# brain-research/l2hmc

Hardware: AMD Instinct MI355X
Metric: chain_leapfrog_steps_per_sec (higher is better)
Workload: dtype f32

## Files before the change

### l2hmc_amd/csrc/traj_fast.hpp

```cpp
#pragma once
#include "l2hmc_kernels.hpp"
#include "bf3k.hpp"


namespace l2hmc {

__device__ __forceinline__ float relu_i(float a) { return __int_as_float(max(__float_as_int(a), 0)); }
__device__ __forceinline__ f4 rcp4(f4 a) {
  return f4{__builtin_amdgcn_rcpf(a.x), __builtin_amdgcn_rcpf(a.y), __builtin_amdgcn_rcpf(a.z),
            __builtin_amdgcn_rcpf(a.w)};
}
__device__ __forceinline__ f4 ex2_4(f4 a) {
  return f4{__builtin_amdgcn_exp2f(a.x), __builtin_amdgcn_exp2f(a.y), __builtin_amdgcn_exp2f(a.z),
            __builtin_amdgcn_exp2f(a.w)};
}

typedef _Float16 h2v __attribute__((ext_vector_type(2)));
typedef _Float16 h8v __attribute__((ext_vector_type(8)));
typedef float f2v __attribute__((ext_vector_type(2)));
#define L2HMC_F16_SCALE 64.0f
struct WF16 {
  h8v a1;
  h8v a2;
};
__device__ __forceinline__ h2v cvt_pk16(float a, float b) { return __builtin_convertvector(f2v{a, b}, h2v); }
__device__ __forceinline__ h2v lo_pair16(h2v h, float a0, float a1) {
  h2v r;
  const float ns = -L2HMC_F16_SCALE;
  asm("v_fma_mixlo_f16 %0, %1, %2, %3 op_sel:[0,0,0] op_sel_hi:[1,0,0]" : "=v"(r) : "v"(h), "s"(ns), "v"(a0));
  asm("v_fma_mixhi_f16 %0, %1, %2, %3 op_sel:[1,0,0] op_sel_hi:[1,0,0]" : "+v"(r) : "v"(h), "s"(ns), "v"(a1));
  return r;
}
template <bool LAT>
__device__ __forceinline__ h8v split16(f4 a) {
  const f4 ad = a * (1.f / L2HMC_F16_SCALE);
  const h2v h01 = cvt_pk16(ad.x, ad.y), h23 = cvt_pk16(ad.z, ad.w);
  h2v l01, l23;
  if constexpr (LAT) {
    float r0, r1, r2, r3;
    const float ns = -L2HMC_F16_SCALE;
    asm("v_fma_mix_f32 %0, %1, %2, %3 op_sel:[0,0,0] op_sel_hi:[1,0,0]" : "=v"(r0) : "v"(h01), "s"(ns), "v"(a.x));
    asm("v_fma_mix_f32 %0, %1, %2, %3 op_sel:[1,0,0] op_sel_hi:[1,0,0]" : "=v"(r1) : "v"(h01), "s"(ns), "v"(a.y));
    asm("v_fma_mix_f32 %0, %1, %2, %3 op_sel:[0,0,0] op_sel_hi:[1,0,0]" : "=v"(r2) : "v"(h23), "s"(ns), "v"(a.z));
    asm("v_fma_mix_f32 %0, %1, %2, %3 op_sel:[1,0,0] op_sel_hi:[1,0,0]" : "=v"(r3) : "v"(h23), "s"(ns), "v"(a.w));
    l01 = cvt_pk16(r0, r1);
    l23 = cvt_pk16(r2, r3);
  } else {
    l01 = lo_pair16(h01, a.x, a.y);
    l23 = lo_pair16(h23, a.z, a.w);
  }
  return h8v{h01.x, h01.y, h23.x, h23.y, l01.x, l01.y, l23.x, l23.y};
}
__device__ __forceinline__ WF16 wsplit16(f4 w) {
  const float sc = L2HMC_F16_SCALE;
  const h2v h01 = cvt_pk16(w.x, w.y), h23 = cvt_pk16(w.z, w.w);
  const f4 r = f4{w.x - (float)h01.x, w.y - (float)h01.y, w.z - (float)h23.x, w.w - (float)h23.y} * sc;
  const h2v L01 = cvt_pk16(r.x, r.y), L23 = cvt_pk16(r.z, r.w);
  const h2v H01 = cvt_pk16((float)h01.x * sc, (float)h01.y * sc), H23 = cvt_pk16((float)h23.x * sc, (float)h23.y * sc);
  const h2v l01 = cvt_pk16((float)L01.x / sc, (float)L01.y / sc), l23 = cvt_pk16((float)L23.x / sc, (float)L23.y / sc);
  WF16 f;
  f.a1 = h8v{H01.x, H01.y, H23.x, H23.y, h01.x, h01.y, h23.x, h23.y};
  f.a2 = h8v{L01.x, L01.y, L23.x, L23.y, l01.x, l01.y, l23.x, l23.y};
  return f;
}
#define L2HMC_F16_STATE_MAX 2.5e5f
__device__ __forceinline__ float amax4(f4 a) { return fmaxf(fmaxf(fabsf(a.x), fabsf(a.y)), fmaxf(fabsf(a.z), fabsf(a.w))); }
__device__ __forceinline__ f4 mfma16x2(const WF16& W, h8v b, f4 acc) {
  acc = __builtin_amdgcn_mfma_f32_16x16x32_f16(W.a1, b, acc, 0, 0, 0);
  return __builtin_amdgcn_mfma_f32_16x16x32_f16(W.a2, b, acc, 0, 0, 0);
}

__host__ __device__ constexpr int fast_fw_net_f32(int NTp) { return (3 * NTp + 1) * 256; }
__host__ __device__ constexpr int fast_fw_net(int NTp, bool f16 = false) { return (3 * NTp + 1) * (f16 ? 512 : 256); }
__host__ __device__ inline int fast_dpp(int NTp) { return 16 * NTp + 16; }
__host__ __device__ inline int fast_fc_net(int NTp) { return 4 * fast_dpp(NTp); }
__host__ __device__ inline int fast_rec(int NTp) { return 32 + 16 * NTp; }
__host__ __device__ inline int fast_rec_dir(int NTp, int T) { return (T + 2) * fast_rec(NTp) + 16; }

long long plan_lds_fast(KArgs& k, int NW, int DT, bool f16 = false);

#ifndef L2HMC_FAST_SPLIT_LAT_TAIL
#define L2HMC_FAST_SPLIT_LAT_TAIL true
#endif
#ifndef L2HMC_FAST_SPLIT_LAT_PAIR
#define L2HMC_FAST_SPLIT_LAT_PAIR true
#endif
#ifndef L2HMC_FAST_SPLIT_LAT_L1
#define L2HMC_FAST_SPLIT_LAT_L1 false
#endif
template <int DT, bool F16 = false>
struct TailK {
  f4 w2;
  f4 hs[DT], ht[DT], hq[DT];
  f4 cS[DT], cQ[DT], bQ[DT];
};
template <int DT>
struct TailK<DT, true> {
  WF16 w2;
  WF16 hs[DT], ht[DT], hq[DT];
  f4 cS[DT], cQ[DT], bQ[DT];
};

template <int DT>
__device__ __forceinline__ void load_tailk(TailK<DT, false>& tk, const float* fw, const float* fc, int dofs, int NTp,
                                           int w, int lane) {
  const int q = lane >> 4, DPp = fast_dpp(NTp);
  tk.w2 = lds4(fw + lane * 4);
#pragma unroll
  for (int t = 0; t < DT; ++t) {
    const int tg = w * DT + t;
    tk.hs[t] = lds4(fw + ((1 + 3 * tg + 0) * 64 + lane) * 4);
    tk.ht[t] = lds4(fw + ((1 + 3 * tg + 1) * 64 + lane) * 4);
    tk.hq[t] = lds4(fw + ((1 + 3 * tg + 2) * 64 + lane) * 4);
    tk.cS[t] = lds4(fc + dofs + 16 * tg + 4 * q);
    tk.cQ[t] = lds4(fc + 2 * DPp + 16 * tg + 4 * q);
    tk.bQ[t] = lds4(fc + 3 * DPp + 16 * tg + 4 * q);
  }
}
__device__ __forceinline__ WF16 lds_wf16(const float* fw, int NTp, int g, int lane) {
  WF16 f;
  f.a1 = *reinterpret_cast<const h8v*>(fw + (g * 64 + lane) * 4);
  f.a2 = *reinterpret_cast<const h8v*>(fw + (3 * NTp + 1) * 256 + (g * 64 + lane) * 4);
  return f;
}
template <int DT>
__device__ __forceinline__ void load_tailk(TailK<DT, true>& tk, const float* fw, const float* fc, int dofs, int NTp,
                                           int w, int lane) {
  const int q = lane >> 4, DPp = fast_dpp(NTp);
  tk.w2 = lds_wf16(fw, NTp, 0, lane);
#pragma unroll
  for (int t = 0; t < DT; ++t) {
    const int tg = w * DT + t;
    tk.hs[t] = lds_wf16(fw, NTp, 1 + 3 * tg + 0, lane);
    tk.ht[t] = lds_wf16(fw, NTp, 1 + 3 * tg + 1, lane);
    tk.hq[t] = lds_wf16(fw, NTp, 1 + 3 * tg + 2, lane);
    tk.cS[t] = lds4(fc + dofs + 16 * tg + 4 * q);
    tk.cQ[t] = lds4(fc + 2 * DPp + 16 * tg + 4 * q);
    tk.bQ[t] = lds4(fc + 3 * DPp + 16 * tg + 4 * q);
  }
}

template <int DT, int KH, class F>
__device__ __forceinline__ void tail_fast(const TailK<DT, false>& tk, f4 hs_, F&& apply) {
  f4 h = splat(0.f);
#pragma unroll
  for (int r = 0; r < KH; ++r) h[r] = relu_i(hs_[r]);
  {
    f4 acc = splat(0.f);
#pragma unroll
    for (int r = 0; r < KH; ++r) acc = MFMA16(tk.w2[r], h[r], acc);
#pragma unroll
    for (int r = 0; r < KH; ++r) h[r] = relu_i(acc[r]);
  }
#pragma unroll
  for (int t = 0; t < DT; ++t) {
    f4 zs = splat(0.f), zt = splat(0.f), zq = splat(0.f);
#pragma unroll
    for (int r = 0; r < KH; ++r) {
      zs = MFMA16(tk.hs[t][r], h[r], zs);
      zq = MFMA16(tk.hq[t][r], h[r], zq);
      zt = MFMA16(tk.ht[t][r], h[r], zt);
    }
#if !defined(L2HMC_NO_HEAD_FENCE)
    __builtin_amdgcn_sched_barrier(0);
#endif
    const f4 rS = rcp4(-(ex2_4(zs) * 0.5f + 0.5f));
    const f4 aS = rS * tk.cS[t] + tk.cS[t];
    const f4 rQ = rcp4(-(ex2_4(zq) * 0.5f + 0.5f));
    const f4 EQ = ex2_4(rQ * tk.cQ[t] + tk.bQ[t]);
    apply(t, aS, zt, EQ);
  }
}
template <int DT, int KH, class F>
__device__ __forceinline__ void tail_fast(const TailK<DT, true>& tk, f4 hs_, F&& apply) {
  f4 h = splat(0.f);
#pragma unroll
  for (int r = 0; r < KH; ++r) h[r] = relu_i(hs_[r]);
  {
    const f4 acc = mfma16x2(tk.w2, split16<L2HMC_FAST_SPLIT_LAT_TAIL>(h), splat(0.f));
#pragma unroll
    for (int r = 0; r < KH; ++r) h[r] = relu_i(acc[r]);
  }
  const h8v b = split16<L2HMC_FAST_SPLIT_LAT_TAIL>(h);
#pragma unroll
  for (int t = 0; t < DT; ++t) {
    f4 zs = __builtin_amdgcn_mfma_f32_16x16x32_f16(tk.hs[t].a1, b, splat(0.f), 0, 0, 0);
    f4 zq = __builtin_amdgcn_mfma_f32_16x16x32_f16(tk.hq[t].a1, b, splat(0.f), 0, 0, 0);
    f4 zt = __builtin_amdgcn_mfma_f32_16x16x32_f16(tk.ht[t].a1, b, splat(0.f), 0, 0, 0);
    zs = __builtin_amdgcn_mfma_f32_16x16x32_f16(tk.hs[t].a2, b, zs, 0, 0, 0);
    zq = __builtin_amdgcn_mfma_f32_16x16x32_f16(tk.hq[t].a2, b, zq, 0, 0, 0);
    zt = __builtin_amdgcn_mfma_f32_16x16x32_f16(tk.ht[t].a2, b, zt, 0, 0, 0);
    const f4 rS = rcp4(-(ex2_4(zs) * 0.5f + 0.5f));
    const f4 aS = rS * tk.cS[t] + tk.cS[t];
    const f4 rQ = rcp4(-(ex2_4(zq) * 0.5f + 0.5f));
    const f4 EQ = ex2_4(rQ * tk.cQ[t] + tk.bQ[t]);
    apply(t, aS, zt, EQ);
  }
}

template <int DT, int KH, class FA, class FB>
__device__ __forceinline__ void tail_fast2(const TailK<DT, true>& tk, f4 hsa, f4 hsb, FA&& applyA, FB&& keepB) {
  f4 ha = splat(0.f), hb = splat(0.f);
#pragma unroll
  for (int r = 0; r < KH; ++r) { ha[r] = relu_i(hsa[r]); hb[r] = relu_i(hsb[r]); }
  {
    const h8v sa = split16<L2HMC_FAST_SPLIT_LAT_PAIR>(ha), sb = split16<L2HMC_FAST_SPLIT_LAT_PAIR>(hb);
    f4 acca = __builtin_amdgcn_mfma_f32_16x16x32_f16(tk.w2.a1, sa, splat(0.f), 0, 0, 0);
    f4 accb = __builtin_amdgcn_mfma_f32_16x16x32_f16(tk.w2.a1, sb, splat(0.f), 0, 0, 0);
    acca = __builtin_amdgcn_mfma_f32_16x16x32_f16(tk.w2.a2, sa, acca, 0, 0, 0);
    accb = __builtin_amdgcn_mfma_f32_16x16x32_f16(tk.w2.a2, sb, accb, 0, 0, 0);
#pragma unroll
    for (int r = 0; r < KH; ++r) { ha[r] = relu_i(acca[r]); hb[r] = relu_i(accb[r]); }
  }
  const h8v ba = split16<L2HMC_FAST_SPLIT_LAT_PAIR>(ha), bb = split16<L2HMC_FAST_SPLIT_LAT_PAIR>(hb);
#pragma unroll
  for (int t = 0; t < DT; ++t) {
    f4 zsa = __builtin_amdgcn_mfma_f32_16x16x32_f16(tk.hs[t].a1, ba, splat(0.f), 0, 0, 0);
    f4 zqa = __builtin_amdgcn_mfma_f32_16x16x32_f16(tk.hq[t].a1, ba, splat(0.f), 0, 0, 0);
    f4 zta = __builtin_amdgcn_mfma_f32_16x16x32_f16(tk.ht[t].a1, ba, splat(0.f), 0, 0, 0);
    f4 zsb = __builtin_amdgcn_mfma_f32_16x16x32_f16(tk.hs[t].a1, bb, splat(0.f), 0, 0, 0);
    f4 zqb = __builtin_amdgcn_mfma_f32_16x16x32_f16(tk.hq[t].a1, bb, splat(0.f), 0, 0, 0);
    f4 ztb = __builtin_amdgcn_mfma_f32_16x16x32_f16(tk.ht[t].a1, bb, splat(0.f), 0, 0, 0);
    zsa = __builtin_amdgcn_mfma_f32_16x16x32_f16(tk.hs[t].a2, ba, zsa, 0, 0, 0);
    zqa = __builtin_amdgcn_mfma_f32_16x16x32_f16(tk.hq[t].a2, ba, zqa, 0, 0, 0);
    zta = __builtin_amdgcn_mfma_f32_16x16x32_f16(tk.ht[t].a2, ba, zta, 0, 0, 0);
    zsb = __builtin_amdgcn_mfma_f32_16x16x32_f16(tk.hs[t].a2, bb, zsb, 0, 0, 0);
    zqb = __builtin_amdgcn_mfma_f32_16x16x32_f16(tk.hq[t].a2, bb, zqb, 0, 0, 0);
    ztb = __builtin_amdgcn_mfma_f32_16x16x32_f16(tk.ht[t].a2, bb, ztb, 0, 0, 0);
    const f4 rSa = rcp4(-(ex2_4(zsa) * 0.5f + 0.5f));
    const f4 aSa = rSa * tk.cS[t] + tk.cS[t];
    const f4 rQa = rcp4(-(ex2_4(zqa) * 0.5f + 0.5f));
    const f4 EQa = ex2_4(rQa * tk.cQ[t] + tk.bQ[t]);
    applyA(t, aSa, zta, EQa);
    const f4 rSb = rcp4(-(ex2_4(zsb) * 0.5f + 0.5f));
    const f4 aSb = rSb * tk.cS[t] + tk.cS[t];
    const f4 rQb = rcp4(-(ex2_4(zqb) * 0.5f + 0.5f));
    const f4 EQb = ex2_4(rQb * tk.cQ[t] + tk.bQ[t]);
    keepB(t, aSb, ztb, EQb);
  }
}

template <int DT>
struct L1W16 {
  WF16 xa[DT], xb[DT], va[DT], vb[DT];
};
template <int DT>
__device__ __forceinline__ f4 l1_part16(const f4 (&z)[DT], f4 acc, const WF16* W) {
#pragma unroll
  for (int t = 0; t < DT; ++t) acc = mfma16x2(W[t], split16<L2HMC_FAST_SPLIT_LAT_L1>(z[t]), acc);
  return acc;
}

template <int EK, int DT, int NW, int KH, int PK = 0>
#ifndef L2HMC_FAST_WAVES
#define L2HMC_FAST_WAVES 2
#endif
#ifndef L2HMC_FAST_WAVES_DT2
#define L2HMC_FAST_WAVES_DT2 1
#endif
__global__ __launch_bounds__(64 * NW, (DT >= 2 && PK == 1) ? L2HMC_FAST_WAVES_DT2 : L2HMC_FAST_WAVES) void traj_fast_kernel(const KArgs A) {
  extern __shared__ __attribute__((aligned(16))) float smem[];
  lds_poison(smem);
  static_assert(DT <= 2, "the fast kernel keeps layer-1 and tail fragments in registers");
  const int tid = threadIdx.x, lane = tid & 63, nthr = 64 * NW;
  const int w = NW > 1 ? __builtin_amdgcn_readfirstlane(tid >> 6) : 0;
  const int c = lane & 15, q = lane >> 4;
  const long long chain = (long long)blockIdx.x * 16 + c;
  const bool live = chain < A.N;
  const int NT = A.NT, DP = 16 * NT, NF = net_floats(NT);
  const float LOG2E = 1.4426950408889634f;
  const float eps = A.alpha != nullptr ? expf(*A.alpha) : A.eps_host;
  const float heps = 0.5f * eps;
  constexpr int NTp = NW * DT;
  constexpr bool F16 = PK == 1;
  const int FWN = fast_fw_net(NTp, F16), DPp = fast_dpp(NTp), FCN = fast_fc_net(NTp), R = fast_rec(NTp),
            RECD = fast_rec_dir(NTp, A.T);

  {
    constexpr int GN = 3 * NTp + 1;
    constexpr int NCP = 2 * GN * 64, NTRIP = (NCP + 64 * NW - 1) / (64 * NW);
    for (int t0 = 0; t0 < NTRIP; t0 += 8) {
      f4 buf[8];
#pragma unroll
      for (int u = 0; u < 8; ++u) {
        const int i = tid + (t0 + u) * nthr;
        const int net = i >= GN * 64, j = i - net * (GN * 64), g = j >> 6;
        buf[u] = splat(0.f);
        if (i < NCP && g < 3 * NT + 1) buf[u] = reinterpret_cast<const f4*>(A.packed + (size_t)net * NF + (2 * NT + 1) * 256)[j];
      }
#pragma unroll
      for (int u = 0; u < 8; ++u) {
        const int i = tid + (t0 + u) * nthr;
        const int net = i >= GN * 64, j = i - net * (GN * 64), g = j >> 6;
        float sc = 1.f;
        if (g > 0) sc = ((g - 1) % 3 == 1) ? (net == 0 ? eps : heps) : 2.f * LOG2E;
        if constexpr (F16) {
          if (i < NCP) {
            const WF16 f = wsplit16(buf[u] * sc);
            float* base = smem + A.o_fw + net * FWN;
            reinterpret_cast<h8v*>(base)[j] = f.a1;
            reinterpret_cast<h8v*>(base + GN * 256)[j] = f.a2;
          }
        } else {
          if (i < NCP) reinterpret_cast<f4*>(smem + A.o_fw + net * FWN)[j] = buf[u] * sc;
        }
      }
    }
  }
  for (int i = tid; i < 2 * 16 * NTp; i += nthr) {
    const int net = i / (16 * NTp), dim = i % (16 * NTp);
    const float* scl = A.packed + (size_t)net * NF + net_groups(NT) * 256;
    const float epn = net == 0 ? eps : heps;
    const float es = dim < DP ? scl[dim] : 0.f, eq = dim < DP ? scl[DP + dim] : 0.f;
    const float cs = es * epn * LOG2E, cq = eq * eps * LOG2E;
    float* fc = smem + A.o_fc + net * FCN;
    fc[dim] = cs;
    fc[DPp + dim] = -cs;
    fc[2 * DPp + dim] = cq;
    fc[3 * DPp + dim] = cq + log2f(epn);
  }
#pragma unroll 4
  for (int i = tid; i < 2 * A.T * R; i += nthr) {
    const int dr = i / (A.T * R), r = (i / R) % A.T, j = i % R;
    const bool tb = j < 32;
    const int net = tb ? j >> 4 : 0, u = j & 15, dim = tb ? 0 : j - 32;
    const float* tf = A.packed + (size_t)net * NF + (2 * NT * 64) * 4;
    const float a0 = tf[u * 4], a1 = tf[(16 + u) * 4], a2 = tf[(32 + u) * 4], c0 = A.trig[2 * r], c1 = A.trig[2 * r + 1];
    const float mk = A.masks[r * A.d + (dim < A.d ? dim : 0)];
    const float m = dim < A.d ? mk : 0.f;
    smem[A.o_rec + dr * RECD + (r + 1) * R + j] = tb ? fmaf(a0, c0, fmaf(a1, c1, a2)) : (dr ? m : 1.f - m);
  }
  stage_energy<EK, false>(A, smem, tid, nthr);

  f4 x[DT], v[DT], g[DT];
  load_state<DT, NW>(A.x, A, chain, live, w, q, x);
  const bool need_p = A.p_out != nullptr || A.x_next != nullptr || A.u != nullptr ||
                      (A.rng_flags & L2HMC_RNG_U) != 0;
  __syncthreads();

  const float* fwx = smem + A.o_fw;
  const float* fwv = fwx + FWN;
  const float* fcx = smem + A.o_fc;
  const float* fcv = fcx + FCN;
  int pb = 0;
  const f4 Z = splat(0.f);
  EnergyRegs<EK, DT> er;
  load_energy_regs<EK, DT, NW>(er, A, smem, w, lane);
  auto grad = [&](const f4 (&xx)[DT], f4 (&gg)[DT], float& Up, bool wantU) {
    if constexpr (EK == L2HMC_ENERGY_GAUSS_DIAG) {
#pragma unroll
      for (int t = 0; t < DT; ++t) gg[t] = er.prec[t] * (xx[t] - er.mu[t]);
    } else {
      grad_energy<EK, DT, NW>(A, smem, w, lane, xx, gg, Up, wantU, &er);
    }
  };
  auto diag_U = [&](const f4 (&xx)[DT], const f4 (&gg)[DT]) {
    float U = 0.f;
    if constexpr (EK == L2HMC_ENERGY_GAUSS_DIAG) {
#pragma unroll
      for (int t = 0; t < DT; ++t) U += 0.5f * hsum((xx[t] - er.mu[t]) * gg[t]);
    }
    return U;
  };
  float U_start = 0.f;
  grad(x, g, U_start, need_p);
  if constexpr (EK == L2HMC_ENERGY_GAUSS_DIAG) U_start = diag_U(x, g);

  L1W<DT> l1w;
  load_l1w<DT, NW>(l1w, A.packed, A.packed + NF, A, w, lane);
  TailK<DT, F16> tk;
  f4 pv[1];
  L1W16<F16 ? DT : 1> l1h;
  auto vnet_l1 = [&](const f4 (&xx)[DT], const f4 (&gg)[DT]) {
    if constexpr (F16) {
      if constexpr (EK == L2HMC_ENERGY_GAUSS_DIAG) return l1_part16<DT>(xx, Z, l1h.va);
      else return l1_part16<DT>(gg, l1_part16<DT>(xx, Z, l1h.va), l1h.vb);
    } else if constexpr (EK == L2HMC_ENERGY_GAUSS_DIAG) {
      return l1_part<DT, NW>(nullptr, 0, A, w, lane, xx, Z, l1w.va);
    } else {
      return l1_part<DT, NW>(nullptr, 0, A, w, lane, xx, Z, l1w.va) + l1_part<DT, NW>(nullptr, NT, A, w, lane, gg, Z, l1w.vb);
    }
  };
  if constexpr (EK == L2HMC_ENERGY_GAUSS_DIAG) {
    f4 pm[DT], cv[1];
#pragma unroll
    for (int t = 0; t < DT; ++t) {
      l1w.va[t] = l1w.va[t] + er.prec[t] * l1w.vb[t];
      pm[t] = -(er.prec[t] * er.mu[t]);
    }
    cv[0] = l1_part<DT, NW>(nullptr, NT, A, w, lane, pm, Z, l1w.vb);
    xchg<NW, 1>(cv, A, smem, w, lane, pb);
    if (w == 0 && c == 0) {
      for (int i = 0; i < 2 * A.T; ++i) {
        float* tb = smem + A.o_rec + (i / A.T) * RECD + (i % A.T + 1) * R + 16 + 4 * q;
        *reinterpret_cast<f4*>(tb) = lds4(tb) + cv[0];
      }
    }
    __syncthreads();
  }
  if constexpr (F16) {
#pragma unroll
    for (int t = 0; t < DT; ++t) {
      l1h.xa[t] = wsplit16(l1w.xa[t]);
      l1h.xb[t] = wsplit16(l1w.xb[t]);
      l1h.va[t] = wsplit16(l1w.va[t]);
      l1h.vb[t] = wsplit16(l1w.vb[t]);
    }
  }
  PT_DECL;
  PT_MARK(0);
  pv[0] = vnet_l1(x, g);
  xchg<NW, 1>(pv, A, smem, w, lane, pb);

  const long long gchain = A.chain_off + chain;
  const bool rng_v = (A.rng_flags & L2HMC_RNG_V) != 0, rng_d = (A.rng_flags & L2HMC_RNG_DIR) != 0;
  const bool rng_u = (A.rng_flags & L2HMC_RNG_U) != 0;
  f4 vn[DT];
  if (!rng_v) load_state<DT, NW>(A.v, A, chain, live, w, q, vn);
  bool fwd_n = (A.dir != nullptr && !rng_d) ? (live ? A.dir[chain] != 0 : true) : (A.dir_all != 0);
  float u_n = (A.u != nullptr && !rng_u && live) ? A.u[chain] : 0.f;
  const bool have_u = A.u != nullptr || rng_u;
  for (int m = 0; m < A.M; ++m) {
    const long long moff = (long long)m * A.N;
    const unsigned long long prop = A.rng_prop0 + (unsigned long long)m;
    if (rng_v) {
      rng_state<DT, NW>(A, gchain, prop, w, q, v);
    } else {
#pragma unroll
      for (int t = 0; t < DT; ++t) v[t] = vn[t];
    }
    bool fwd = fwd_n;
    float u_m = u_n;
    if (rng_d || rng_u) {
      bool fr;
      float ur;
      philox_dir_u(A.rng_seed, gchain, prop, fr, ur);
      if (rng_d) fwd = fr;
      if (rng_u) u_m = ur;
    }
    if (m + 1 < A.M) {
      if (!rng_v) load_state<DT, NW>(A.v + (moff + A.N) * A.d, A, chain, live, w, q, vn);
      if (A.dir != nullptr && !rng_d && live) fwd_n = A.dir[moff + A.N + chain] != 0;
      if (A.u != nullptr && !rng_u && live) u_n = A.u[moff + A.N + chain];
    }
    constexpr bool KEEP_G0 = EK != L2HMC_ENERGY_GAUSS_DIAG;
    f4 x0[DT], g0[KEEP_G0 ? DT : 1];
#pragma unroll
    for (int t = 0; t < DT; ++t) {
      x0[t] = x[t];
      if constexpr (KEEP_G0) g0[t] = g[t];
    }
    const f4 pv0 = pv[0];
    float red[F16 ? 6 : 5];
    float amax_l = 0.f;
    if constexpr (F16) {
#pragma unroll
      for (int t = 0; t < DT; ++t) amax_l = fmaxf(amax_l, fmaxf(amax4(x[t]), fmaxf(amax4(v[t]), amax4(g[t]))));
    }
    red[0] = U_start;
    red[1] = 0.f;
#pragma unroll
    for (int t = 0; t < DT; ++t) red[1] += 0.5f * hsum(v[t] * v[t]);
    red[2] = 0.f;
    f4 ldv = splat(0.f);

    const float ff = fwd ? 1.f : 0.f, nf = ff - 1.f;
    const int dofs = fwd ? 0 : DPp;
    const int row0 = fwd ? A.step_begin : (A.T - 1 - A.step_begin);
    const float* rec = smem + A.o_rec + (fwd ? RECD : 0) + (row0 + 1) * R + 4 * q;
    const int drec = fwd ? R : -R;
    f4 tbv = lds4(rec + 16);

    constexpr bool RT = DT == 1 || PK == 1;
    TailK<DT, F16> tkx;
    if constexpr (RT) load_tailk<DT>(tkx, fwx, fcx, dofs, NTp, w, lane);
    const TailK<DT, F16>& TKX = *(RT ? &tkx : &tk);
    load_tailk<DT>(tk, fwv, fcv, dofs, NTp, w, lane);
#ifndef L2HMC_FAST_SERIAL_TAILS
#ifndef L2HMC_FAST_PAIR_DT2
#define L2HMC_FAST_PAIR_DT2 0
#endif
    constexpr bool PAIR = F16 && RT && (DT == 1 || L2HMC_FAST_PAIR_DT2);
#else
    constexpr bool PAIR = false;
#endif
    f4 aS_n[DT], T_n[DT], EQ_n[DT];
    if constexpr (PAIR) {
      tail_fast<DT, KH>(tk, pv[0] + tbv, [&](int t, f4 aS, f4 T, f4 EQ) { aS_n[t] = aS; T_n[t] = T; EQ_n[t] = EQ; });
    }
    for (int it = 0; it < A.n_steps; ++it) {
      f4 k1[DT], vh[DT], y[DT], xin[DT];
      const f4 tbx = lds4(rec);
#pragma unroll
      for (int t = 0; t < DT; ++t) k1[t] = lds4(rec + 32 + 16 * (w * DT + t));
      rec += drec;
      const f4 tbv_n = lds4(rec + 16);

      PT_MARK(1);
      auto vhalf1 = [&](int t, f4 aS, f4 T, f4 EQ) {
        const f4 ES = ex2_4(aS);
        ldv += aS;
        const f4 tr = T - EQ * g[t];
        vh[t] = ES * (nf * tr + v[t]) + ff * tr;
      };
      if constexpr (PAIR) {
#pragma unroll
        for (int t = 0; t < DT; ++t) vhalf1(t, aS_n[t], T_n[t], EQ_n[t]);
      } else {
        tail_fast<DT, KH>(tk, pv[0] + tbv, vhalf1);
      }
      PT_MARK(2);

      if constexpr (!RT) load_tailk<DT>(tk, fwx, fcx, dofs, NTp, w, lane);
#pragma unroll
      for (int t = 0; t < DT; ++t) xin[t] = k1[t] * x[t];
      f4 pa, px[1];
      if constexpr (F16) {
        pa = l1_part16<DT>(vh, Z, l1h.xa);
        px[0] = l1_part16<DT>(xin, pa, l1h.xb);
      } else {
        pa = l1_part<DT, NW>(nullptr, 0, A, w, lane, vh, Z, l1w.xa);
        px[0] = pa + l1_part<DT, NW>(nullptr, NT, A, w, lane, xin, Z, l1w.xb);
      }
      PT_MARK(3);
      xchg<NW, 1>(px, A, smem, w, lane, pb);
      PT_MARK(4);
      tail_fast<DT, KH>(TKX, px[0] + tbx, [&](int t, f4 aS, f4 T, f4 EQ) {
        const f4 up = 1.f - k1[t];
        const f4 aSm = up * aS;
        const f4 ES = ex2_4(aSm);
        ldv += aSm;
        const f4 tr = up * (EQ * vh[t] + T);
        y[t] = ES * (nf * tr + x[t]) + ff * tr;
        xin[t] = up * y[t];
      });
      PT_MARK(5);
      f4 py[1];
      if constexpr (F16) py[0] = l1_part16<DT>(xin, pa, l1h.xb);
      else py[0] = pa + l1_part<DT, NW>(nullptr, NT, A, w, lane, xin, Z, l1w.xb);
      PT_MARK(6);
      xchg<NW, 1>(py, A, smem, w, lane, pb);
      PT_MARK(7);
      tail_fast<DT, KH>(TKX, py[0] + tbx, [&](int t, f4 aS, f4 T, f4 EQ) {
        const f4 aSm = k1[t] * aS;
        const f4 ES = ex2_4(aSm);
        ldv += aSm;
        const f4 tr = k1[t] * (EQ * vh[t] + T);
        x[t] = ES * (nf * tr + y[t]) + ff * tr;
      });
      PT_MARK(8);

      if constexpr (!RT) load_tailk<DT>(tk, fwv, fcv, dofs, NTp, w, lane);
      grad(x, g, red[2], need_p && it == A.n_steps - 1);
      pv[0] = vnet_l1(x, g);
      PT_MARK(9);
      xchg<NW, 1>(pv, A, smem, w, lane, pb);
      PT_MARK(10);
      auto vhalf2 = [&](int t, f4 aS, f4 T, f4 EQ) {
        const f4 ES = ex2_4(aS);
        ldv += aS;
        const f4 tr = T - EQ * g[t];
        v[t] = ES * (nf * tr + vh[t]) + ff * tr;
      };
      if constexpr (PAIR) {
        tail_fast2<DT, KH>(tk, pv[0] + tbv, pv[0] + tbv_n, vhalf2, [&](int t, f4 aS, f4 T, f4 EQ) { aS_n[t] = aS; T_n[t] = T; EQ_n[t] = EQ; });
      } else {
        tail_fast<DT, KH>(tk, pv[0] + tbv, vhalf2);
      }
      PT_MARK(11);
      tbv = tbv_n;
    }
    if constexpr (EK == L2HMC_ENERGY_GAUSS_DIAG) red[2] = diag_U(x, g);
    const float ld = hsum(ldv) * 0.6931471805599453f;

    const bool last = m == A.M - 1;
    red[3] = 0.f;
#pragma unroll
    for (int t = 0; t < DT; ++t) red[3] += 0.5f * hsum(v[t] * v[t]);
    red[4] = ld;
    const float U_end = red[2];
    if constexpr (F16) {
#pragma unroll
      for (int t = 0; t < DT; ++t) amax_l = fmaxf(amax_l, fmaxf(amax4(x[t]), fmaxf(amax4(v[t]), amax4(g[t]))));
      red[5] = amax_l < L2HMC_F16_STATE_MAX ? 0.f : 1.f;
    }
    chain_allreduce<NW, F16 ? 6 : 5>(red, smem + A.o_red, w, lane);
    if constexpr (F16) {
      if (red[5] > 0.f) {
        const float qnan = __uint_as_float(0x7fc00000u);
#pragma unroll
        for (int t = 0; t < DT; ++t) { x[t] = splat(qnan); v[t] = splat(qnan); }
        red[4] = qnan;
      }
    }
    if (last) {
      store_state<DT, NW>(A.x_out, A, chain, live, w, q, x);
      store_state<DT, NW>(A.v_out, A, chain, live, w, q, v);
    }
    const bool writer = live && w == 0 && lane < 16;
    if (A.logjac_out != nullptr && writer) A.logjac_out[moff + chain] = red[4];
    if (need_p) {
      const float val = (red[0] + red[1]) - (red[2] + red[3]) + red[4];
      const float p = accept_prob(val);
      if (A.p_out != nullptr && writer) A.p_out[moff + chain] = p;
      if (have_u) {
        const bool acc = live && (p - u_m) >= 0.f;
#pragma unroll
        for (int t = 0; t < DT; ++t) {
          x[t] = sel4(acc, x[t], x0[t]);
          if constexpr (KEEP_G0) g[t] = sel4(acc, g[t], g0[t]);
          else g[t] = er.prec[t] * (x[t] - er.mu[t]);
        }
        pv[0] = sel4(acc, pv[0], pv0);
        U_start = acc ? U_end : U_start;
      } else {
        U_start = U_end;
      }
    } else {
      U_start = U_end;
    }
    if (A.x_hist != nullptr) store_state<DT, NW>(A.x_hist + moff * A.d, A, chain, live, w, q, x);
  }
  PT_FLUSH(w, lane);
  store_state<DT, NW>(A.x_next, A, chain, live, w, q, x);
}

}
```

Measured before the change: 2.353 billion.

## Specialize fast kernel for common config, peel last leapfrog step, parallelize setup

Adds a compile-time 'common config' variant of the fast trajectory kernel for Gaussian-diag, DT=1, paired mode, so runtime flag checks and unused output paths are removed. It peels the last leapfrog step so the paired tail does not compute a discarded next-step prediction, and skips the fourth split residual when KH==3. It also restructures the per-block record setup into batched, unrolled loads split by section, spreads the bias fold across 16 lanes, and moves state and L1 weight loads earlier to overlap with setup. This adds code size and template instantiations, which may raise register pressure.

After: 2.418 billion, median of 6. 2.7% higher.

```diff
diff --git a/l2hmc_amd/csrc/traj_fast.hpp b/l2hmc_amd/csrc/traj_fast.hpp
--- a/l2hmc_amd/csrc/traj_fast.hpp
+++ b/l2hmc_amd/csrc/traj_fast.hpp
@@ -31,18 +31,18 @@
   asm("v_fma_mixhi_f16 %0, %1, %2, %3 op_sel:[1,0,0] op_sel_hi:[1,0,0]" : "+v"(r) : "v"(h), "s"(ns), "v"(a1));
   return r;
 }
-template <bool LAT>
+template <bool LAT, bool W0 = false>
 __device__ __forceinline__ h8v split16(f4 a) {
   const f4 ad = a * (1.f / L2HMC_F16_SCALE);
   const h2v h01 = cvt_pk16(ad.x, ad.y), h23 = cvt_pk16(ad.z, ad.w);
   h2v l01, l23;
   if constexpr (LAT) {
-    float r0, r1, r2, r3;
+    float r0, r1, r2, r3 = 0.f;
     const float ns = -L2HMC_F16_SCALE;
     asm("v_fma_mix_f32 %0, %1, %2, %3 op_sel:[0,0,0] op_sel_hi:[1,0,0]" : "=v"(r0) : "v"(h01), "s"(ns), "v"(a.x));
     asm("v_fma_mix_f32 %0, %1, %2, %3 op_sel:[1,0,0] op_sel_hi:[1,0,0]" : "=v"(r1) : "v"(h01), "s"(ns), "v"(a.y));
     asm("v_fma_mix_f32 %0, %1, %2, %3 op_sel:[0,0,0] op_sel_hi:[1,0,0]" : "=v"(r2) : "v"(h23), "s"(ns), "v"(a.z));
-    asm("v_fma_mix_f32 %0, %1, %2, %3 op_sel:[1,0,0] op_sel_hi:[1,0,0]" : "=v"(r3) : "v"(h23), "s"(ns), "v"(a.w));
+    if constexpr (!W0) asm("v_fma_mix_f32 %0, %1, %2, %3 op_sel:[1,0,0] op_sel_hi:[1,0,0]" : "=v"(r3) : "v"(h23), "s"(ns), "v"(a.w));
     l01 = cvt_pk16(r0, r1);
     l23 = cvt_pk16(r2, r3);
   } else {
@@ -177,11 +177,11 @@
 #pragma unroll
   for (int r = 0; r < KH; ++r) h[r] = relu_i(hs_[r]);
   {
-    const f4 acc = mfma16x2(tk.w2, split16<L2HMC_FAST_SPLIT_LAT_TAIL>(h), splat(0.f));
+    const f4 acc = mfma16x2(tk.w2, split16<L2HMC_FAST_SPLIT_LAT_TAIL, KH == 3>(h), splat(0.f));
 #pragma unroll
     for (int r = 0; r < KH; ++r) h[r] = relu_i(acc[r]);
   }
-  const h8v b = split16<L2HMC_FAST_SPLIT_LAT_TAIL>(h);
+  const h8v b = split16<L2HMC_FAST_SPLIT_LAT_TAIL, KH == 3>(h);
 #pragma unroll
   for (int t = 0; t < DT; ++t) {
     f4 zs = __builtin_amdgcn_mfma_f32_16x16x32_f16(tk.hs[t].a1, b, splat(0.f), 0, 0, 0);
@@ -204,7 +204,7 @@
 #pragma unroll
   for (int r = 0; r < KH; ++r) { ha[r] = relu_i(hsa[r]); hb[r] = relu_i(hsb[r]); }
   {
-    const h8v sa = split16<L2HMC_FAST_SPLIT_LAT_PAIR>(ha), sb = split16<L2HMC_FAST_SPLIT_LAT_PAIR>(hb);
+    const h8v sa = split16<L2HMC_FAST_SPLIT_LAT_PAIR, KH == 3>(ha), sb = split16<L2HMC_FAST_SPLIT_LAT_PAIR, KH == 3>(hb);
     f4 acca = __builtin_amdgcn_mfma_f32_16x16x32_f16(tk.w2.a1, sa, splat(0.f), 0, 0, 0);
     f4 accb = __builtin_amdgcn_mfma_f32_16x16x32_f16(tk.w2.a1, sb, splat(0.f), 0, 0, 0);
     acca = __builtin_amdgcn_mfma_f32_16x16x32_f16(tk.w2.a2, sa, acca, 0, 0, 0);
@@ -212,7 +212,7 @@
 #pragma unroll
     for (int r = 0; r < KH; ++r) { ha[r] = relu_i(acca[r]); hb[r] = relu_i(accb[r]); }
   }
-  const h8v ba = split16<L2HMC_FAST_SPLIT_LAT_PAIR>(ha), bb = split16<L2HMC_FAST_SPLIT_LAT_PAIR>(hb);
+  const h8v ba = split16<L2HMC_FAST_SPLIT_LAT_PAIR, KH == 3>(ha), bb = split16<L2HMC_FAST_SPLIT_LAT_PAIR, KH == 3>(hb);
 #pragma unroll
   for (int t = 0; t < DT; ++t) {
     f4 zsa = __builtin_amdgcn_mfma_f32_16x16x32_f16(tk.hs[t].a1, ba, splat(0.f), 0, 0, 0);
@@ -251,6 +251,9 @@
   return acc;
 }
 
+template <int EK, int DT, int NW, int KH, int PK, bool CC>
+__device__ __forceinline__ void traj_fast_body(const KArgs& A);
+
 template <int EK, int DT, int NW, int KH, int PK = 0>
 #ifndef L2HMC_FAST_WAVES
 #define L2HMC_FAST_WAVES 2
@@ -259,6 +262,19 @@
 #define L2HMC_FAST_WAVES_DT2 1
 #endif
 __global__ __launch_bounds__(64 * NW, (DT >= 2 && PK == 1) ? L2HMC_FAST_WAVES_DT2 : L2HMC_FAST_WAVES) void traj_fast_kernel(const KArgs A) {
+  if constexpr (EK == L2HMC_ENERGY_GAUSS_DIAG && DT == 1 && PK == 1) {
+    const bool common = (A.rng_flags & (L2HMC_RNG_V | L2HMC_RNG_DIR | L2HMC_RNG_U)) == (L2HMC_RNG_V | L2HMC_RNG_DIR | L2HMC_RNG_U) &&
+                        A.p_out != nullptr && A.x_next != nullptr && A.x_hist == nullptr && A.logjac_out == nullptr &&
+                        A.x_out == nullptr && A.v_out == nullptr;
+    if (common) traj_fast_body<EK, DT, NW, KH, PK, true>(A);
+    else traj_fast_body<EK, DT, NW, KH, PK, false>(A);
+  } else {
+    traj_fast_body<EK, DT, NW, KH, PK, false>(A);
+  }
+}
+
+template <int EK, int DT, int NW, int KH, int PK, bool CC>
+__device__ __forceinline__ void traj_fast_body(const KArgs& A) {
   extern __shared__ __attribute__((aligned(16))) float smem[];
   lds_poison(smem);
   static_assert(DT <= 2, "the fast kernel keeps layer-1 and tail fragments in registers");
@@ -276,6 +292,10 @@
   const int FWN = fast_fw_net(NTp, F16), DPp = fast_dpp(NTp), FCN = fast_fc_net(NTp), R = fast_rec(NTp),
             RECD = fast_rec_dir(NTp, A.T);
 
+  f4 x[DT], v[DT], g[DT];
+  load_state<DT, NW>(A.x, A, chain, live, w, q, x);
+  L1W<DT> l1w;
+  load_l1w<DT, NW>(l1w, A.packed, A.packed + NF, A, w, lane);
   {
     constexpr int GN = 3 * NTp + 1;
     constexpr int NCP = 2 * GN * 64, NTRIP = (NCP + 64 * NW - 1) / (64 * NW);
@@ -319,22 +339,52 @@
     fc[2 * DPp + dim] = cq;
     fc[3 * DPp + dim] = cq + log2f(epn);
   }
-#pragma unroll 4
-  for (int i = tid; i < 2 * A.T * R; i += nthr) {
-    const int dr = i / (A.T * R), r = (i / R) % A.T, j = i % R;
-    const bool tb = j < 32;
-    const int net = tb ? j >> 4 : 0, u = j & 15, dim = tb ? 0 : j - 32;
-    const float* tf = A.packed + (size_t)net * NF + (2 * NT * 64) * 4;
-    const float a0 = tf[u * 4], a1 = tf[(16 + u) * 4], a2 = tf[(32 + u) * 4], c0 = A.trig[2 * r], c1 = A.trig[2 * r + 1];
-    const float mk = A.masks[r * A.d + (dim < A.d ? dim : 0)];
-    const float m = dim < A.d ? mk : 0.f;
-    smem[A.o_rec + dr * RECD + (r + 1) * R + j] = tb ? fmaf(a0, c0, fmaf(a1, c1, a2)) : (dr ? m : 1.f - m);
+  constexpr int SU = 4;
+  {
+    const int nA = A.T * 32;
+    for (int i0 = tid; i0 < nA; i0 += SU * nthr) {
+      float a0[SU], a1[SU], a2[SU], c0[SU], c1[SU];
+#pragma unroll
+      for (int s = 0; s < SU; ++s) {
+        const int i = min(i0 + s * nthr, nA - 1), r = i >> 5, net = (i >> 4) & 1, u = i & 15;
+        const float* tf = A.packed + (size_t)net * NF + (2 * NT * 64) * 4;
+        a0[s] = tf[u * 4], a1[s] = tf[(16 + u) * 4], a2[s] = tf[(32 + u) * 4], c0[s] = A.trig[2 * r], c1[s] = A.trig[2 * r + 1];
+      }
+#pragma unroll
+      for (int s = 0; s < SU; ++s) {
+        const int i = i0 + s * nthr, r = i >> 5, j = i & 31;
+        if (i < nA) {
+          const float tbr = fmaf(a0[s], c0[s], fmaf(a1[s], c1[s], a2[s]));
+          smem[A.o_rec + (r + 1) * R + j] = tbr;
+          smem[A.o_rec + RECD + (r + 1) * R + j] = tbr;
+        }
+      }
+    }
+  }
+  {
+    constexpr int W16 = 16 * NTp;
+    const int nB = A.T * W16;
+    for (int i0 = tid; i0 < nB; i0 += SU * nthr) {
+      float mk[SU];
+#pragma unroll
+      for (int s = 0; s < SU; ++s) {
+        const int i = min(i0 + s * nthr, nB - 1), r = i / W16, dim = i % W16;
+        mk[s] = A.masks[r * A.d + (dim < A.d ? dim : 0)];
+      }
+#pragma unroll
+      for (int s = 0; s < SU; ++s) {
+        const int i = i0 + s * nthr, r = i / W16, dim = i % W16;
+        if (i < nB) {
+          const float m = dim < A.d ? mk[s] : 0.f;
+          smem[A.o_rec + (r + 1) * R + 32 + dim] = 1.f - m;
+          smem[A.o_rec + RECD + (r + 1) * R + 32 + dim] = m;
+        }
+      }
+    }
   }
   stage_energy<EK, false>(A, smem, tid, nthr);
 
-  f4 x[DT], v[DT], g[DT];
-  load_state<DT, NW>(A.x, A, chain, live, w, q, x);
-  const bool need_p = A.p_out != nullptr || A.x_next != nullptr || A.u != nullptr ||
+  const bool need_p = CC || A.p_out != nullptr || A.x_next != nullptr || A.u != nullptr ||
                       (A.rng_flags & L2HMC_RNG_U) != 0;
   __syncthreads();
 
@@ -366,8 +416,6 @@
   grad(x, g, U_start, need_p);
   if constexpr (EK == L2HMC_ENERGY_GAUSS_DIAG) U_start = diag_U(x, g);
 
-  L1W<DT> l1w;
-  load_l1w<DT, NW>(l1w, A.packed, A.packed + NF, A, w, lane);
   TailK<DT, F16> tk;
   f4 pv[1];
   L1W16<F16 ? DT : 1> l1h;
@@ -390,8 +438,8 @@
     }
     cv[0] = l1_part<DT, NW>(nullptr, NT, A, w, lane, pm, Z, l1w.vb);
     xchg<NW, 1>(cv, A, smem, w, lane, pb);
-    if (w == 0 && c == 0) {
-      for (int i = 0; i < 2 * A.T; ++i) {
+    if (w == 0) {
+      for (int i = c; i < 2 * A.T; i += 16) {
         float* tb = smem + A.o_rec + (i / A.T) * RECD + (i % A.T + 1) * R + 16 + 4 * q;
         *reinterpret_cast<f4*>(tb) = lds4(tb) + cv[0];
       }
@@ -413,13 +461,13 @@
   xchg<NW, 1>(pv, A, smem, w, lane, pb);
 
   const long long gchain = A.chain_off + chain;
-  const bool rng_v = (A.rng_flags & L2HMC_RNG_V) != 0, rng_d = (A.rng_flags & L2HMC_RNG_DIR) != 0;
-  const bool rng_u = (A.rng_flags & L2HMC_RNG_U) != 0;
+  const bool rng_v = CC || (A.rng_flags & L2HMC_RNG_V) != 0, rng_d = CC || (A.rng_flags & L2HMC_RNG_DIR) != 0;
+  const bool rng_u = CC || (A.rng_flags & L2HMC_RNG_U) != 0;
   f4 vn[DT];
   if (!rng_v) load_state<DT, NW>(A.v, A, chain, live, w, q, vn);
   bool fwd_n = (A.dir != nullptr && !rng_d) ? (live ? A.dir[chain] != 0 : true) : (A.dir_all != 0);
   float u_n = (A.u != nullptr && !rng_u && live) ? A.u[chain] : 0.f;
-  const bool have_u = A.u != nullptr || rng_u;
+  const bool have_u = CC || A.u != nullptr || rng_u;
   for (int m = 0; m < A.M; ++m) {
     const long long moff = (long long)m * A.N;
     const unsigned long long prop = A.rng_prop0 + (unsigned long long)m;
@@ -488,7 +536,8 @@
     if constexpr (PAIR) {
       tail_fast<DT, KH>(tk, pv[0] + tbv, [&](int t, f4 aS, f4 T, f4 EQ) { aS_n[t] = aS; T_n[t] = T; EQ_n[t] = EQ; });
     }
-    for (int it = 0; it < A.n_steps; ++it) {
+    auto step = [&](auto LASTC, bool wantU) {
+      constexpr bool LAST = decltype(LASTC)::value;
       f4 k1[DT], vh[DT], y[DT], xin[DT];
       const f4 tbx = lds4(rec);
 #pragma unroll
@@ -551,7 +600,7 @@
       PT_MARK(8);
 
       if constexpr (!RT) load_tailk<DT>(tk, fwv, fcv, dofs, NTp, w, lane);
-      grad(x, g, red[2], need_p && it == A.n_steps - 1);
+      grad(x, g, red[2], wantU);
       pv[0] = vnet_l1(x, g);
       PT_MARK(9);
       xchg<NW, 1>(pv, A, smem, w, lane, pb);
@@ -563,12 +612,22 @@
         v[t] = ES * (nf * tr + vh[t]) + ff * tr;
       };
       if constexpr (PAIR) {
-        tail_fast2<DT, KH>(tk, pv[0] + tbv, pv[0] + tbv_n, vhalf2, [&](int t, f4 aS, f4 T, f4 EQ) { aS_n[t] = aS; T_n[t] = T; EQ_n[t] = EQ; });
+        if constexpr (!LAST) {
+          tail_fast2<DT, KH>(tk, pv[0] + tbv, pv[0] + tbv_n, vhalf2, [&](int t, f4 aS, f4 T, f4 EQ) { aS_n[t] = aS; T_n[t] = T; EQ_n[t] = EQ; });
+        } else {
+          tail_fast<DT, KH>(tk, pv[0] + tbv, vhalf2);
+        }
       } else {
         tail_fast<DT, KH>(tk, pv[0] + tbv, vhalf2);
       }
       PT_MARK(11);
       tbv = tbv_n;
+    };
+    if constexpr (PAIR && EK == L2HMC_ENERGY_GAUSS_DIAG) {
+      for (int it = 0; it + 1 < A.n_steps; ++it) step(std::false_type{}, false);
+      if (A.n_steps > 0) step(std::true_type{}, need_p);
+    } else {
+      for (int it = 0; it < A.n_steps; ++it) step(std::false_type{}, need_p && it == A.n_steps - 1);
     }
     if constexpr (EK == L2HMC_ENERGY_GAUSS_DIAG) red[2] = diag_U(x, g);
     const float ld = hsum(ldv) * 0.6931471805599453f;
@@ -593,16 +652,16 @@
         red[4] = qnan;
       }
     }
-    if (last) {
+    if (!CC && last) {
       store_state<DT, NW>(A.x_out, A, chain, live, w, q, x);
       store_state<DT, NW>(A.v_out, A, chain, live, w, q, v);
     }
     const bool writer = live && w == 0 && lane < 16;
-    if (A.logjac_out != nullptr && writer) A.logjac_out[moff + chain] = red[4];
+    if (!CC && A.logjac_out != nullptr && writer) A.logjac_out[moff + chain] = red[4];
     if (need_p) {
       const float val = (red[0] + red[1]) - (red[2] + red[3]) + red[4];
       const float p = accept_prob(val);
-      if (A.p_out != nullptr && writer) A.p_out[moff + chain] = p;
+      if ((CC || A.p_out != nullptr) && writer) A.p_out[moff + chain] = p;
       if (have_u) {
         const bool acc = live && (p - u_m) >= 0.f;
 #pragma unroll
@@ -619,7 +678,7 @@
     } else {
       U_start = U_end;
     }
-    if (A.x_hist != nullptr) store_state<DT, NW>(A.x_hist + moff * A.d, A, chain, live, w, q, x);
+    if (!CC && A.x_hist != nullptr) store_state<DT, NW>(A.x_hist + moff * A.d, A, chain, live, w, q, x);
   }
   PT_FLUSH(w, lane);
   store_state<DT, NW>(A.x_next, A, chain, live, w, q, x);
```
